# rsmedleystevenson/pyamg

Hardware: AMD Instinct MI355X
Metric: V-cycle iterations/sec (3D Poisson 500^3 fp64, SA-AMG, chebyshev smoother) (higher is better)
Workload: dtype f64; 1 GPU; 3D Poisson 500x500x500 (125.0M dof, nnz 873.5M) CSR fp64, smoothed aggregation (5 levels), Chebyshev degree 2 pre/post smoother, V(1,1), b=rand seed 0; parallelism=single GPU

## Files before the change

include/amgcore_hip.h:

```cpp
#ifndef AMGCORE_HIP_H
#define AMGCORE_HIP_H

#ifdef __cplusplus
extern "C" {
#endif

#define AMG_OK        0
#define AMG_EINVAL   -1
#define AMG_ENODEV   -2
#define AMG_ENOMEM   -3
#define AMG_ESTATE   -4
#define AMG_ENOTIMPL -5

const char *amg_last_error(void);
int amg_device_count(void);
const char *amg_device_name(int device);



int amgcore_gauss_seidel_f64(const int Ap[], int Ap_size, const int Aj[], int Aj_size,
                             const double Ax[], int Ax_size, double x[], int x_size,
                             const double b[], int b_size,
                             int row_start, int row_stop, int row_step);
int amgcore_bsr_gauss_seidel_f64(const int Ap[], int Ap_size, const int Aj[], int Aj_size,
// ... 150 lines not shown
int amg_hier_set_matrix(amg_hier *h, int lvl, int which, int fmt, int nrows, int ncols,
                        int R, int C, const int *Ap, const int *Aj, const double *Ax,
                        int on_device);
int amg_hier_set_smoother(amg_hier *h, int lvl, int which, const amg_smoother_desc *d);
int amg_hier_set_block_matrix(amg_hier *h, int lvl, int which, int nbrows, int bs, const int *Ap,
                              const int *Aj, const double *Ax);
int amg_hier_set_aux_matrix(amg_hier *h, int lvl, int which, int slot, int nmajor, int nminor,
                            const int *Ap, const int *Aj, const double *Ax);
int amg_hier_set_coarse_dense(amg_hier *h, const double *M, int n);
int amg_hier_set_coarse_smoother(amg_hier *h, const amg_smoother_desc *d);
int amg_hier_set_callback_smoother(amg_hier *h, int lvl, int which, amg_relax_callback cb, void *user);
int amg_hier_set_coarse_callback(amg_hier *h, amg_coarse_callback cb, void *user);
int amg_hier_apply(amg_hier *h, int lvl, int which, const double *x_dev, double *y_dev);
int amg_hier_apply_aux(amg_hier *h, int lvl, int which, int slot, const double *x_dev, double *y_dev);
double *amg_hier_scratch(amg_hier *h);
int amg_hier_finalize(amg_hier *h);
long amg_hier_release_sources(amg_hier *h);

int amg_hier_solve(amg_hier *h, const double *b, double *x, double tol, int maxiter, int cycle,
                   double *residuals, int *nres, int flags);
int amg_hier_pcg(amg_hier *h, const double *b, double *x, double tol, int maxiter, int cycle,
                 double *residuals, int *nres, int *info, int flags);
int amg_hier_cycle(amg_hier *h, const double *b, double *x, int cycle, int flags);
int amg_hier_relax(amg_hier *h, int lvl, int which, const double *b, double *x);
int amg_hier_matvec(amg_hier *h, int lvl, int which, const double *x, double *y);

double amg_hier_cycle_bytes(amg_hier *h, int cycle);
int amg_hier_operator_form(amg_hier *h, int lvl);
int amg_hier_value_index(amg_hier *h, int lvl, int on);
void amg_set_value_index(int on);
int amg_value_index_enabled(void);
void amg_set_level0_fusion(int on);
int amg_hier_level0_fused(amg_hier *h);
int amg_hier_gs_natural(amg_hier *h, int lvl, double *x, const double *b, const unsigned char *dirs, int nsweeps);

double amg_hier_operator_bytes(amg_hier *h, int lvl, int moved);
double amg_hier_cycle_bytes_moved(amg_hier *h, int cycle);
double amg_hier_last_solve_ms(amg_hier *h);
long amg_hier_device_bytes(amg_hier *h);
void *amg_hier_stream(amg_hier *h);
double *amg_hier_dev_x(amg_hier *h);
double *amg_hier_dev_b(amg_hier *h);

int amg_hier_time_spmv(amg_hier *h, int lvl, int which, int mode, int reps, double *ms);
int amg_hier_time_relax(amg_hier *h, int lvl, int which, int reps, double *ms);

typedef struct amg_mat amg_mat;
amg_mat *amg_mat_create(int device, int nrows, int ncols, const int *Ap, const int *Aj, const double *Ax);
void amg_mat_destroy(amg_mat *m);
long amg_mat_nnz(amg_mat *m);
int amg_mat_form(amg_mat *m);
int amg_mat_apply(amg_mat *m, int mode, const double *xg, const double *b, const double *v2, double *out,
                  double *out2, double c0, double gscale, void *stream);
int amg_mat_apply_rows(amg_mat *m, int mode, int row_lo, int row_hi, const double *xg, const double *b,
                       const double *v2, double *out, double *out2, double c0, double gscale, void *stream);
int amg_mat_build_gs(amg_mat *m, const int *order, int norder);
int amg_mat_gs_levels(amg_mat *m);
int amg_mat_gs_sweep(amg_mat *m, double *x, const double *b, int reverse, int bsr1, void *stream);
int amg_mat_gs_sweeps(amg_mat *m, double *x, const double *b, const unsigned char *seq, int nseq, int bsr1, void *stream);
int amg_dev_scale(double *out, const double *in, double c, long n, void *stream);
int amg_dev_axpy(double *x, const double *h, long n, void *stream);
int amg_dev_axpy_scaled(double *x, const double *r, double c, long n, void *stream);
int amg_dev_norm2(const double *x, long n, double *scratch, double *result_dev, void *stream);
int amg_dev_dot(const double *x, const double *y, long n, double *scratch, double *result_dev, void *stream);
int amg_dev_dense_apply(const double *Mt, const double *b, double *x, int n, void *stream);
int amg_dev_gather(double *out, const double *in, const int *idx, long n, void *stream);
// ... 146 lines not shown
```

pyamg_amd/_lib.py:

```python
import ctypes as C
import os

import numpy as np

HERE = os.path.dirname(os.path.abspath(__file__))
LIB_PATH = os.environ.get("AMGCORE_HIP_LIB") or os.path.join(HERE, "lib", "libamgcore_hip.so")

c_int_p = C.POINTER(C.c_int)
c_dbl_p = C.POINTER(C.c_double)

AMG_OK, AMG_EINVAL, AMG_ENODEV, AMG_ENOMEM, AMG_ESTATE, AMG_ENOTIMPL = 0, -1, -2, -3, -4, -5


class AmgError(RuntimeError):
    pass


class AmgDeviceError(AmgError):
    pass


RELAX_CALLBACK = C.CFUNCTYPE(C.c_int, C.c_void_p, C.c_int, C.c_void_p, C.c_void_p)
COARSE_CALLBACK = C.CFUNCTYPE(C.c_int, C.c_void_p, C.c_int, c_dbl_p, c_dbl_p)

# ... 179 lines not shown
    L.amg_hier_destroy.restype = None
    L.amg_hierx_destroy.argtypes = [V]
    L.amg_hierx_destroy.restype = None
    L.amg_hierx_device_bytes.argtypes = [V]
    L.amg_hierx_device_bytes.restype = C.c_long
    L.amg_hierx_last_solve_ms.argtypes = [V]
    L.amg_hierx_last_solve_ms.restype = D
    L.amg_hierx_stream.argtypes = [V]
    L.amg_hierx_stream.restype = V
    L.amg_hierx_scratch.argtypes = [V]
    L.amg_hierx_scratch.restype = V
    L.amg_hierx_level_size.argtypes = [V, I]
    L.amg_hierx_level_size.restype = I
    L.amg_hierx_vec_alloc.argtypes = [V, C.c_long]
    L.amg_hierx_vec_alloc.restype = V
    L.amg_hierx_vec_free.argtypes = [V, V, C.c_long]
    L.amg_hierx_vec_free.restype = None
    L.amg_hierm_destroy.argtypes = [V]
    L.amg_hierm_destroy.restype = None
    L.amg_hierm_device_bytes.argtypes = [V]
    L.amg_hierm_device_bytes.restype = C.c_long
    L.amg_hierm_last_solve_ms.argtypes = [V]
    L.amg_hierm_last_solve_ms.restype = D
    L.amg_hier_cycle_bytes.argtypes = [V, I]
    L.amg_hier_cycle_bytes.restype = D
    L.amg_hier_value_index.argtypes = [V, I, I]
    L.amg_hier_value_index.restype = I
    L.amg_set_value_index.argtypes = [I]
    L.amg_set_value_index.restype = None
    L.amg_set_level0_fusion.argtypes = [I]
    L.amg_set_level0_fusion.restype = None
    L.amg_hier_level0_fused.argtypes = [V]
    L.amg_hier_level0_fused.restype = I
    L.amg_value_index_enabled.argtypes = []
    L.amg_value_index_enabled.restype = I
    L.amg_hier_gs_natural.argtypes = [V, I, V, V, V, I]
    L.amg_hier_gs_natural.restype = I
    L.amg_hier_operator_form.argtypes = [V, I]
    L.amg_hier_operator_form.restype = I
    L.amg_hier_operator_bytes.argtypes = [V, I, I]
    L.amg_hier_operator_bytes.restype = D
    L.amg_hier_cycle_bytes_moved.argtypes = [V, I]
    L.amg_hier_cycle_bytes_moved.restype = D
    L.amg_hier_last_solve_ms.argtypes = [V]
    L.amg_hier_last_solve_ms.restype = D
    L.amg_hier_device_bytes.argtypes = [V]
    L.amg_hier_device_bytes.restype = C.c_long
    L.amg_hier_stream.argtypes = [V]
    L.amg_hier_stream.restype = V
    L.amg_hier_dev_x.argtypes = [V]
    L.amg_hier_dev_x.restype = V
    L.amg_hier_dev_b.argtypes = [V]
    L.amg_hier_dev_b.restype = V
    L.amg_dev_alloc.argtypes = [C.c_long]
    L.amg_dev_alloc.restype = V
    L.amg_dev_free.argtypes = [V]
    L.amg_dev_free.restype = None
    L.amg_hier_scratch.argtypes = [V]
    L.amg_hier_scratch.restype = V
    L.amg_comm_create.argtypes = [I, I, I, I]
    L.amg_comm_create.restype = V
    L.amg_comm_destroy.argtypes = [V]
    L.amg_comm_destroy.restype = None
    L.amg_hier_release_sources.argtypes = [V]
    L.amg_hier_release_sources.restype = C.c_long
    L.amg_mat_create.argtypes = [I, I, I, c_int_p, c_int_p, c_dbl_p]
# ... 77 lines not shown
```

pyamg_amd/csrc/amg_dev.hpp:

```cpp
#pragma once
#include <hip/hip_runtime.h>
#include <cstdint>
#include <string>
#include <vector>

namespace amg {

void set_error(const std::string &msg);
int hip_fail(hipError_t e, const char *what, const char *file, int line);
#define AMG_HIP(call)                                                         \
    do {                                                                      \
        hipError_t e__ = (call);                                              \
        if (e__ != hipSuccess) return amg::hip_fail(e__, #call, __FILE__, __LINE__); \
    } while (0)

constexpr int PAD = 16;

struct DevBsr;
struct DevCsr {
    int nrows = 0, ncols = 0;
    long nnz = 0;
    int *Ap = nullptr;
    int *Aj = nullptr;
    double *Ax = nullptr;
// ... 6 lines not shown
    int npat = 0, ndict = 0;
    int period_rows = 0;
    int *sl_row = nullptr;
    unsigned short *sl_len = nullptr;
    long *sl_off = nullptr;
    int *sl_col = nullptr;
    double *sl_val = nullptr;
    int sl_nslices = 0;
    unsigned *sl_code = nullptr;
    int *sl_org = nullptr;
    long *sl_coff = nullptr;
    unsigned char *sl_flag16 = nullptr;
    double sl_frac16 = 0.0;
    long sl_entries = 0;
    int sl_lo = 0, sl_hi = 0;
    double *st_vals = nullptr;
    void *st_mask = nullptr;
    int st_nu = 0;
    int st_nranges = 0;
    int st_range[8][2] = {{0}};
    unsigned char *st_codes = nullptr;
    double *st_dict = nullptr;
    int st_ndict = 0;
    bool st_vi_on = false;
    unsigned short *Aj16 = nullptr;
    int *wg_base = nullptr;
    unsigned char *wg_flag = nullptr;
    int i16_rpb = 0;
    double i16_frac = 0.0;
    int st_u0 = -1;
    int st_off[32] = {0};
    int l0_ok = 0;
    int l0_nx = 0, l0_ny = 0, l0_nz = 0;
};
constexpr int STENCIL_MAX = 31;
constexpr int STENCIL_RANGES = 8;

constexpr int PAT_MAX = 255;
constexpr int PAT_DICT_MAX = 2048;

struct DevBsr {
    int nbrows = 0, bs = 1;
    long nblocks = 0;
    int *Ap = nullptr;
    int *Aj = nullptr;
    double *Ax = nullptr;
    int *bsl_brow = nullptr;
    unsigned short *bsl_len = nullptr;
    long *bsl_off = nullptr;
    int *bsl_col = nullptr;
    double *bsl_val = nullptr;
    int bsl_nslices = 0;
};

enum StreamMode {
    SM_MATVEC = 0,
    SM_MATVEC_ACC,
    SM_RESIDUAL,
    SM_POLY_FIRST,
    SM_POLY_STEP,
    SM_POLY_LAST,
    SM_JACOBI,
    SM_JACOBI_BSR1,
    SM_GS,
    SM_GS_BSR1,
    SM_RESIDUAL_SUMSQ,
// ... 15 lines not shown
    long nnz_total;
    int rows_per_wg;
    const unsigned short *Aj16;
    const int *wg_base;
    const unsigned char *wg_flag;
    double gscale;
};

int launch_stream(StreamMode mode, const StreamArgs &a, hipStream_t st);
int launch_pattern(StreamMode mode, const StreamArgs &a, const DevCsr &M, hipStream_t st);
bool pattern_supports(StreamMode mode);
int launch_stencil(StreamMode mode, const StreamArgs &a, const DevCsr &M, hipStream_t st);
bool sell_supports(StreamMode mode);
bool sell_enabled();
void set_sell_form(int on);
void set_sell_index16(int on);
bool sell_index16_enabled();
int launch_sell(StreamMode mode, const StreamArgs &a, const DevCsr &M, hipStream_t st);
int build_sell(DevCsr &M, long *acct, int row_lo = 0, int row_hi = -1);
void free_sell(DevCsr &M);
int stencil_blocks(const StreamArgs &a, const DevCsr &M);
struct Level0ChainArgs {
    const unsigned long long *codes;
    const double *dict;
    int ndict;
    int nx, ny, nz;
    const double *g0;
    const double *x;
    const double *b;
    double *xout, *rout;
    double c_gs, c_last;
    int zc;
    int tiles_x, tiles_y;
};
int launch_level0_chain(bool first_res, bool last_res, const Level0ChainArgs &a, hipStream_t st);
int level0_chain_tile(int stages, int axis);
int level0_chain_lanes(int axis);
int launch_sumsq_partials(const double *r, int n, double *out2, hipStream_t st);
int launch_level0_box_scan(const unsigned char *codes, int nx, int ny, int nz, int *bad, hipStream_t st);
int launch_stencil_build(const DevCsr &M, const int *dict_slot, const unsigned *pat_mask, hipStream_t st);
int launch_value_scan(const double *vals, long count, unsigned long long *table, int *overflow, hipStream_t st);
int launch_value_encode(const double *vals, long count, const double *dict_sorted, int ndict, unsigned char *codes, int nu,
                        hipStream_t st, const unsigned char *mask8 = nullptr, long nrows = 0);
int config_epoch();
void bump_config_epoch();
int launch_gs_chain(const DevCsr &G, const int *rowmap, const int *diagpos, const int *level_ptr_dev, int l_first,
                    int nlevels, int width, bool reverse, bool bsr1, double *x, const double *b, hipStream_t st);
constexpr int CHAIN2_WG = 512;
constexpr int CHAIN2_PF = 12;
constexpr int CHAIN2_D = 2;
constexpr int CHAIN2_LMAX = 4096;
constexpr int CHAIN2_EMPTY = -2147483647 - 1;
int launch_perm_gather(const int *rowmap, const double *x, const double *b, const double *diag, double *xp, double *bp, double *bd,
                       int n, hipStream_t st);
int launch_perm_scatter(const int *rowmap, const double *xp, double *x, int n, hipStream_t st);
int launch_gs_chain2(const int *lp, const double *val, const int *code, const int *off, double *dummy, int pf,
                     int l_first, int nlevels, int width, bool reverse, bool bsr1, double *x, const double *bd, int nzero, hipStream_t st);
int gs_chain_max_rows();
int launch_gs_chain_long(const DevCsr &G, const int *rowmap, const int *diagpos, const int *level_ptr_dev, int l_first,
                         int nlevels, int width, bool reverse, bool bsr1, double *x, const double *b, hipStream_t st,
                         const int *ring_code = nullptr);
int gs_chainl_max_levels();
int launch_gs_level(const StreamArgs &a, bool bsr1, const int *gp_host, hipStream_t st);
void set_gs_level_hint(int on);
int gs_chainl_max_rows();
int gs_chainl_entries_per_lane();
bool gs_chain_enabled();
int gs_chain_generation();
void set_gs_chain(int on);
bool stencil_enabled();
int launch_index16_build(DevCsr &M, int rpb, hipStream_t st);
bool index16_enabled();
// ... 115 lines not shown
```

pyamg_amd/csrc/hier.hip:

```cpp
#include <array>
#include <thread>
#include "hier.hpp"

#include <algorithm>
#include <cmath>
#include <cstdlib>
#include <cstring>

namespace amg {

static thread_local std::string g_err;
void set_error(const std::string &msg) { g_err = msg; }
const std::string &last_error() { return g_err; }
int hip_fail(hipError_t e, const char *what, const char *file, int line)
{
    g_err = std::string("HIP error: ") + hipGetErrorString(e) + " in " + what + " (" + file + ":" +
            std::to_string(line) + ")";
    return (e == hipErrorOutOfMemory) ? AMG_ENOMEM : AMG_ENODEV;
}

#define CHK(call)                 \
    do {                          \
        int rc__ = (call);        \
        if (rc__ != 0) return rc__; \
    } while (0)

template <class T> static int dev_alloc(T **p, long count, long *acct)
{
    size_t bytes = sizeof(T) * (size_t)(count + PAD);
    AMG_HIP(hipMalloc((void **)p, bytes));
    AMG_HIP(hipMemset(*p, 0, bytes));
    AMG_HIP(hipDeviceSynchronize());
    if (acct) *acct += (long)bytes;
    return 0;
}

void free_csr(DevCsr &M)
{
    if (M.Ap) hipFree(M.Ap);
    if (M.Aj) hipFree(M.Aj);
    if (M.Ax) hipFree(M.Ax);
    if (M.pat) hipFree(M.pat);
    if (M.dict_ptr) hipFree(M.dict_ptr);
    if (M.dict_off) hipFree(M.dict_off);
    free_sell(M);
    if (M.st_vals) hipFree(M.st_vals);
    if (M.st_mask) hipFree(M.st_mask);
    if (M.st_codes) hipFree(M.st_codes);
    if (M.st_dict) hipFree(M.st_dict);
    if (M.Aj16) hipFree(M.Aj16);
    if (M.wg_base) hipFree(M.wg_base);
    if (M.wg_flag) hipFree(M.wg_flag);
    M = DevCsr();
}
static void free_bsr(DevBsr &M)
{
    free_bsell(M);
    if (M.Ap) hipFree(M.Ap);
    if (M.Aj) hipFree(M.Aj);
    if (M.Ax) hipFree(M.Ax);
    M = DevBsr();
}

int upload_csr(DevCsr &M, int nrows, int ncols, const int *Ap, const int *Aj, const double *Ax,
               long *acct)
{
    long nnz = Ap[nrows];
    if (nnz < 0 || nrows < 0) { set_error("row pointer overflows int32 (more than 2^31-1 stored entries)"); return AMG_EINVAL; }
    M.nrows = nrows; M.ncols = ncols; M.nnz = nnz;
    CHK(dev_alloc(&M.Ap, nrows + 1, acct));
    CHK(dev_alloc(&M.Aj, nnz, acct));
    CHK(dev_alloc(&M.Ax, nnz, acct));
    AMG_HIP(hipMemcpy(M.Ap, Ap, sizeof(int) * (size_t)(nrows + 1), hipMemcpyHostToDevice));
    if (nnz) {
        AMG_HIP(hipMemcpy(M.Aj, Aj, sizeof(int) * (size_t)nnz, hipMemcpyHostToDevice));
        AMG_HIP(hipMemcpy(M.Ax, Ax, sizeof(double) * (size_t)nnz, hipMemcpyHostToDevice));
    }
    return 0;
}

int build_index16(DevCsr &M, const int *Ap_host, long *acct)
{
// ... 1087 lines not shown
}

static int coarse_solve(amg_hier *h, const double *b, double *&x, double *&xalt)
{
    Level &L = h->lv[h->nlevels - 1];
    const int n = L.A.nrows;
    if (L.A.nnz == 0 || h->coarse_kind == 0) {
        AMG_HIP(hipMemsetAsync(x, 0, sizeof(double) * (size_t)n, h->stream));
        return 0;
    }
    if (h->coarse_kind == 1 && h->comm && h->coarse_gather_channel >= 0) {
        CHK(comm_exchange_begin(h->comm, h->coarse_gather_channel, b, h->coarse_gather_idx, h->coarse_full_b, h->stream));
        CHK(comm_exchange_end(h->comm, h->coarse_gather_channel, h->coarse_full_b, h->stream));
        CHK(launch_dense_apply(h->coarse_Mt, h->coarse_full_b, h->coarse_full_x, h->coarse_n, h->stream));
        AMG_HIP(hipMemcpyAsync(x, h->coarse_full_x + h->coarse_lo, sizeof(double) * (size_t)n, hipMemcpyDeviceToDevice, h->stream));
        return 0;
    }
    if (h->coarse_kind == 1) return launch_dense_apply(h->coarse_Mt, b, x, n, h->stream);
    if (h->coarse_kind == 3) {
        h->coarse_hb.resize((size_t)n); h->coarse_hx.assign((size_t)n, 0.0);
        AMG_HIP(hipMemcpyAsync(h->coarse_hb.data(), b, sizeof(double) * (size_t)n, hipMemcpyDeviceToHost, h->stream));
        AMG_HIP(hipStreamSynchronize(h->stream));
        if (h->coarse_cb(h->coarse_cb_user, n, h->coarse_hb.data(), h->coarse_hx.data()) != 0) { set_error("coarse solver callback failed"); return AMG_ESTATE; }
        AMG_HIP(hipMemcpyAsync(x, h->coarse_hx.data(), sizeof(double) * (size_t)n, hipMemcpyHostToDevice, h->stream));
        AMG_HIP(hipStreamSynchronize(h->stream));
        return 0;
    }
    if (h->comm && L.part.channel >= 0) { set_error("relaxation as coarse solver has no row-partitioned form"); return AMG_ENOTIMPL; }
    AMG_HIP(hipMemsetAsync(x, 0, sizeof(double) * (size_t)n, h->stream));
    return relax(h, L, h->coarse_sm, x, xalt, b, true);
}

static int g_level0_fusion = 1;
#ifndef L0_ZCHUNK_PLANES
#define L0_ZCHUNK_PLANES 128
#endif
constexpr int L0_ZCHUNK = L0_ZCHUNK_PLANES;

static int level0_chain_check(amg_hier *h, DevCsr &M)
{
    M.l0_ok = 0;
    if (!M.st_vals || !M.st_codes || M.st_nu != 7 || M.st_nranges != 0 || M.nrows != M.ncols || M.nrows < 1) return 0;
    const int *o = M.st_off;
    const long n = M.nrows, Lx = o[5], P = o[6];
    if (!(o[0] == -P && o[1] == -Lx && o[2] == -1 && o[3] == 0 && o[4] == 1)) return 0;
    if (!(Lx > 1 && P > Lx && P % Lx == 0 && n % P == 0)) return 0;
    int *bad = nullptr;
    if (dev_alloc(&bad, 1, nullptr) != 0) return AMG_ENOMEM;
    int found = 1;
    int rc = 0;
    if (hipMemsetAsync(bad, 0, sizeof(int), h->stream) != hipSuccess) rc = AMG_ESTATE;
    if (rc == 0) rc = launch_level0_box_scan(M.st_codes, (int)Lx, (int)(P / Lx), (int)(n / P), bad, h->stream);
    if (rc == 0 && (hipMemcpyAsync(&found, bad, sizeof(int), hipMemcpyDeviceToHost, h->stream) != hipSuccess ||
                    hipStreamSynchronize(h->stream) != hipSuccess)) rc = AMG_ESTATE;
    hipFree(bad);
    if (rc != 0) return rc;
    if (found) return 0;
    M.l0_nx = (int)Lx; M.l0_ny = (int)(P / Lx); M.l0_nz = (int)(n / P);
    M.l0_ok = 1;
    return 0;
}

static bool level0_fused(amg_hier *h)
{
    if (!g_level0_fusion || h->comm || h->nlevels < 2) return false;
    const Level &L = h->lv[0];
    const DevCsr &M = L.A;
    if (!M.l0_ok || !M.st_vi_on || !M.st_codes || (M.blk && M.blk->Ap) || !(stencil_enabled() || !M.Ap)) return false;
    for (int w = 0; w < 2; ++w) {
        const Smoother &s = L.sm[w];
        if (s.kind != AMG_SM_POLYNOMIAL || s.coef.size() != 2 || s.iterations != 1) return false;
    }
    return true;
}

static int level0_chain(amg_hier *h, const Smoother &s, bool first_res, bool last_res, const double *g0, double *&x,
                        double *&xalt, const double *b, double *rout)
{
    const DevCsr &M = h->lv[0].A;
    Level0ChainArgs a{};
    a.codes = reinterpret_cast<const unsigned long long *>(M.st_codes);
    a.dict = M.st_dict; a.ndict = M.st_ndict;
    a.nx = M.l0_nx; a.ny = M.l0_ny; a.nz = M.l0_nz;
    a.g0 = g0; a.x = x; a.b = b; a.xout = xalt; a.rout = rout;
    a.c_gs = s.coef[0]; a.c_last = s.coef[1];
    a.zc = std::min(L0_ZCHUNK, M.l0_nz);
    CHK(launch_level0_chain(first_res, last_res, a, h->stream));
    std::swap(x, xalt);
    return 0;
}

static int level0_pre_chain(amg_hier *h, double *&x, double *&xalt, const double *b, bool x_zero, bool r_ready)
{
    Level &L = h->lv[0];
    if (x_zero) return level0_chain(h, L.sm[AMG_PRE], false, true, b, x, xalt, b, L.h);
    if (r_ready) return level0_chain(h, L.sm[AMG_PRE], false, true, L.r, x, xalt, b, L.h);
    return level0_chain(h, L.sm[AMG_PRE], true, true, x, x, xalt, b, L.h);
}

static int level0_post_chain(amg_hier *h, double *&x, double *&xalt, const double *b)
{
    Level &L = h->lv[0];
    const bool norm = h->norm_next;
    CHK(level0_chain(h, L.sm[AMG_POST], true, norm, x, x, xalt, b, norm ? L.r : nullptr));
    h->r_fresh = norm;
    return 0;
}

static int cycle(amg_hier *h, int lvl, double *&x, double *&xalt, const double *b, int cyc, bool x_zero,
                 bool r_ready = false)
{
    Level &L = h->lv[lvl];
    Level &Lc = h->lv[lvl + 1];
    hipStream_t st = h->stream;
    const int nc = Lc.A.nrows;
    const bool fused = lvl == 0 && level0_fused(h);

    double *rr = L.r;
    if (fused) {
// ... 1131 lines not shown
        const double f16 = (M.sl_code && sell_index16_enabled()) ? M.sl_frac16 : 0.0;
        return (12.0 - 2.0 * f16) * (double)M.sl_entries + (6.0 * 64.0 + 64.0 * f16 + 1.0) * M.sl_nslices + 8.0 * (M.sl_nslices + 1.0) + 8.0 * M.ncols + 8.0 * M.nrows;
    }
    if (!M.pat) {
        double idx = (M.Aj16 && index16_enabled()) ? (2.0 * M.i16_frac + 4.0 * (1.0 - M.i16_frac)) : 4.0;
        return (8.0 + idx) * (double)M.nnz + 4.0 * (M.nrows + 1.0) + 8.0 * M.ncols + 8.0 * M.nrows;
    }
    return 8.0 * (double)M.nnz + 4.0 * M.nrows + 4.0 * (M.nrows + 1.0) + 8.0 * M.ncols + 8.0 * M.nrows;
}

static double cycle_bytes_impl(amg_hier *h, int cyc, bool moved)
{
    if (!h) return 0.0;
    std::vector<double> visits((size_t)h->nlevels, 0.0);
    visits[0] = 1.0;
    for (int l = 1; l < h->nlevels; ++l) {
        if (cyc == AMG_CYCLE_W) visits[l] = 2.0 * visits[l - 1];
        else if (cyc == AMG_CYCLE_F) visits[l] = visits[l - 1] + 1.0;
        else visits[l] = 1.0;
    }
    double total = 0.0;
    for (int l = 0; l < h->nlevels - 1; ++l) {
        Level &L = h->lv[l];
        double n = L.A.nrows;
        double app = (moved ? bytes_spmv_moved(L.A) : bytes_spmv(L.A)) + 8.0 * n;
        double k = smoother_apps(L.sm[0], l > 0) + 1.0 + smoother_apps(L.sm[1], false);
        double extra = 0.0;
        if (l == 0 && moved && level0_fused(h)) {
            const double zc = std::min(L0_ZCHUNK, L.A.l0_nz);
            const double tx = level0_chain_lanes(0), ty = level0_chain_lanes(1);
            auto chain = [&](int S, int row_operands, int outputs) {
                const double in = (double)level0_chain_tile(S, 0) * level0_chain_tile(S, 1);
                const double zf = (zc + 2.0 * S) / zc;
                return 8.0 * n * (tx * ty / in * zf + row_operands * (tx - 2.0) * (ty - 2.0) / in * zf + outputs);
            };
            const bool kept = h->keep_residual != 0;
            const double pre = kept ? chain(2, 3, 2) : chain(3, 2, 2);
            const double post = chain(3, 2, 2) + 8.0 * n;
            total += visits[l] * (pre + post + bytes_spmv(L.Rm) + bytes_spmv(L.P) + 8.0 * n);
            continue;
        }
        if (l == 0) {
            k += 1.0;
            if (moved && h->keep_residual && L.sm[0].kind == AMG_SM_POLYNOMIAL && L.sm[0].iterations >= 1) {
                k -= 1.0;
                extra = 8.0 * n;
            }
        }
        total += visits[l] * (k * app + extra + bytes_spmv(L.Rm) + bytes_spmv(L.P) + 8.0 * n);
    }
    double ncs = h->lv[h->nlevels - 1].A.nrows;
    total += visits[h->nlevels - 1] * (8.0 * ncs * ncs + 16.0 * ncs);
    return total;
}

int amg_hier_value_index(amg_hier *h, int lvl, int on)
{
    ENTER(h);
    if (lvl < 0 || lvl >= h->nlevels) { set_error("bad level"); return AMG_EINVAL; }
    DevCsr &M = h->lv[lvl].A;
    if (on < 0) return (M.st_vi_on && M.st_codes) ? M.st_ndict : 0;
    drop_graphs(h);
    if (!on) { M.st_vi_on = false; return 0; }
    return value_index_build(h, M);
}

int amg_hier_operator_form(amg_hier *h, int lvl)
{
    if (!h || lvl < 0 || lvl >= h->nlevels) return -1;
    const DevCsr &M = h->lv[lvl].A;
    if (M.st_vals && (stencil_enabled() || !M.Ap)) return 2;
// ... 268 lines not shown
    Level &L = h->lv[lvl];
    Smoother &s = (which == 2) ? h->coarse_sm : L.sm[which];
    CHK(relax(h, L, s, L.x, L.xalt, L.b, false));
    AMG_HIP(hipEventRecord(h->ev0, h->stream));
    for (int r = 0; r < reps; ++r) CHK(relax(h, L, s, L.x, L.xalt, L.b, false));
    AMG_HIP(hipEventRecord(h->ev1, h->stream));
    AMG_HIP(hipStreamSynchronize(h->stream));
    float t = 0.f;
    AMG_HIP(hipEventElapsedTime(&t, h->ev0, h->ev1));
    *ms = t / reps;
    return 0;
}

void amg_set_stream_variant(int v) { amg::set_stream_variant(v); }
void amg_set_stream_pipe(int on) { amg::set_stream_pipe(on); }
void amg_set_xcd_chunk(int c) { amg::set_xcd_chunk(c); }
void amg_set_xcd_period(int on) { amg::set_xcd_period(on); }
void amg_set_stencil_form(int on) { amg::set_stencil_form(on); }
void amg_set_stencil_pairs(int on) { amg::set_stencil_pairs(on); }
void amg_set_sell_form(int on) { amg::set_sell_form(on); }
void amg_set_sell_index16(int on) { amg::set_sell_index16(on); }
void amg_set_gs_chain(int on) { amg::set_gs_chain(on); }
void amg_set_gs_level_hint(int on) { amg::set_gs_level_hint(on); }
void amg_set_gs_flow(int mode) { amg::set_gs_flow(mode); }
void amg_set_gs_flow_lookahead(int levels) { amg::set_gs_flow_lookahead(levels); }
int amg_gs_flow_status(void) { return amg::gs_flow_status(); }
void amg_set_bsr_spmv(int on) { amg::set_bsr_spmv(on); }
void amg_set_index16(int on) { amg::set_index16(on); }
void amg_set_tile_target(int t) { amg::set_tile_target(t); }
void amg_hier_use_graphs(amg_hier *h, int on) { if (h) { h->use_graphs = on; if (!on) drop_graphs(h); } }
void amg_hier_keep_residual(amg_hier *h, int on) { if (h) { h->keep_residual = on; h->r_kept = false; drop_graphs(h); } }
void amg_set_level0_fusion(int on) { g_level0_fusion = on ? 1 : 0; amg::bump_config_epoch(); }
int amg_hier_level0_fused(amg_hier *h) { return (h && h->finalized && level0_fused(h)) ? 1 : 0; }

}
```

pyamg_amd/csrc/kernels.hip:

```cpp
#include "amg_dev.hpp"

namespace amg {

constexpr int WG = 256;
#ifndef AMG_TILE
#define AMG_TILE 2048
#endif
constexpr int TILE = AMG_TILE;

typedef int v4i __attribute__((ext_vector_type(4)));
typedef double v2d __attribute__((ext_vector_type(2)));
__device__ __forceinline__ v4i load_v4i(const int *p)
{
#ifdef AMG_NT_LOADS
    return __builtin_nontemporal_load(reinterpret_cast<const v4i *>(p));
#else
    return *reinterpret_cast<const v4i *>(p);
#endif
}
__device__ __forceinline__ v2d load_v2d(const double *p)
{
#ifdef AMG_NT_LOADS
    return __builtin_nontemporal_load(reinterpret_cast<const v2d *>(p));
#else
    return *reinterpret_cast<const v2d *>(p);
#endif
}

static int g_stream_variant = 1;
static int g_xcd_chunk = 32;
static int g_tile_target = 2048;
static int g_config_epoch = 0;
int config_epoch() { return g_config_epoch; }
// ... 1856 lines not shown
        c.row_hi = std::min(a.row_hi, M.st_range[r][1]);
        if (c.row_hi <= c.row_lo) continue;
        if (MODE == SM_RESIDUAL_SUMSQ) c.out2 = a.out2 + done;
        int rc = launch_pattern((StreamMode)MODE, c, M, st);
        if (rc != 0) return rc;
        done += (c.row_hi - c.row_lo + rpb - 1) / rpb;
    }
    return 0;
}

int launch_stencil(StreamMode mode, const StreamArgs &a, const DevCsr &M, hipStream_t st)
{
    switch (mode) {
    case SM_MATVEC: return launch_stencil_mode<SM_MATVEC>(a, M, st);
    case SM_MATVEC_ACC: return launch_stencil_mode<SM_MATVEC_ACC>(a, M, st);
    case SM_RESIDUAL: return launch_stencil_mode<SM_RESIDUAL>(a, M, st);
    case SM_POLY_STEP: return launch_stencil_mode<SM_POLY_STEP>(a, M, st);
    case SM_POLY_LAST: return launch_stencil_mode<SM_POLY_LAST>(a, M, st);
    case SM_JACOBI: return launch_stencil_mode<SM_JACOBI>(a, M, st);
    case SM_JACOBI_BSR1: return launch_stencil_mode<SM_JACOBI_BSR1>(a, M, st);
    case SM_RESIDUAL_SUMSQ: return launch_stencil_mode<SM_RESIDUAL_SUMSQ>(a, M, st);
    default: break;
    }
    set_error("launch_stencil: mode not supported");
    return -1;
}

#ifndef L0C_TY
#define L0C_TY 16
#endif
constexpr int L0C_TX = 32;
constexpr int L0C_WG = L0C_TX * L0C_TY;
constexpr int L0C_PAD = L0C_TX;

template <int FR, int LR>
__global__ __launch_bounds__(L0C_WG) void level0_chain_kernel(Level0ChainArgs a)
{
    constexpr int S = FR + 1 + LR;
    constexpr int SP = FR + 1;
    constexpr int INX = L0C_TX - 2 * S, INY = L0C_TY - 2 * S;
    __shared__ double sdict[256];
    __shared__ double pl[2][S][L0C_WG + 2 * L0C_PAD];
    const int t = threadIdx.x, tx = t % L0C_TX, ty = t / L0C_TX;
    const int bid = remap_block(blockIdx.x, gridDim.x, 16);
    const int tiles = a.tiles_x * a.tiles_y;
    const int zb = bid / tiles, rem = bid - zb * tiles;
    const int tyi = rem / a.tiles_x, txi = rem - tyi * a.tiles_x;
    const int gx = txi * INX - S + tx, gy = tyi * INY - S + ty;
    const bool inxy = gx >= 0 && gx < a.nx && gy >= 0 && gy < a.ny;
    const bool ring1 = inxy && tx >= 1 && tx < L0C_TX - 1 && ty >= 1 && ty < L0C_TY - 1;
    const bool inner = inxy && tx >= S && tx < L0C_TX - S && ty >= S && ty < L0C_TY - S;
    const long P = (long)a.nx * a.ny;
    const long col = inxy ? (long)gy * a.nx + gx : 0;
    const int z0 = zb * a.zc, z1 = min(z0 + a.zc, a.nz);
    if (t < a.ndict) sdict[t] = a.dict[t];

    double w[S + 1][3];
    unsigned long long cq[S];
    double bq[S];
#pragma unroll
    for (int s = 0; s <= S; ++s) w[s][0] = w[s][1] = w[s][2] = 0.0;
#pragma unroll
    for (int s = 0; s < S; ++s) { cq[s] = ~0ULL; bq[s] = 0.0; }
    double xq = 0.0;
    int k = z0 - S;
    double g_next = (inxy && k >= 0) ? a.g0[(long)k * P + col] : 0.0;
    unsigned long long c_next = ~0ULL;
    double b_next = 0.0, x_next = 0.0;
    const int iters = (z1 - z0) + 2 * S;
    for (int j = 0; j < iters; ++j, ++k) {
        w[0][0] = w[0][1]; w[0][1] = w[0][2]; w[0][2] = g_next;
#pragma unroll
        for (int s = S - 1; s > 0; --s) { cq[s] = cq[s - 1]; bq[s] = bq[s - 1]; }
        cq[0] = c_next; bq[0] = b_next; xq = x_next;
        {
            const int kn = k + 1;
            g_next = (inxy && kn >= 0 && kn < a.nz) ? a.g0[(long)kn * P + col] : 0.0;
            const bool rowk = ring1 && k >= 0 && k < a.nz;
            const long ik = (long)k * P + col;
            c_next = rowk ? a.codes[ik] : ~0ULL;
            b_next = rowk ? a.b[ik] : 0.0;
            if (!FR) x_next = rowk ? a.x[ik] : 0.0;
        }
        double (*plb)[L0C_WG + 2 * L0C_PAD] = pl[j & 1];
#pragma unroll
        for (int s = 1; s <= S; ++s) plb[s - 1][L0C_PAD + t] = s == 1 ? w[0][1] : w[s - 1][2];
        __syncthreads();
#pragma unroll
        for (int s = 1; s <= S; ++s) {
            const double *q = &plb[s - 1][L0C_PAD + t];
            const double xv[7] = {w[s - 1][0], q[-L0C_TX], q[-1], w[s - 1][1], q[1], q[L0C_TX], w[s - 1][2]};
            double diag = 0.0, val;
            if (s == SP) {
                const double acc = coded_row_sum<SM_POLY_LAST>(cq[s - 1], sdict, xv, a.c_gs, true, 0.0, -1, diag);
                val = poly_last_row(a.c_last, w[s - 1][1], acc, FR ? w[0][0] : xq);
            } else {
                const double acc = coded_row_sum<SM_RESIDUAL>(cq[s - 1], sdict, xv, 1.0, true, 0.0, -1, diag);
                val = residual_row(bq[s - 1], acc);
            }
            w[s][0] = w[s][1]; w[s][1] = w[s][2]; w[s][2] = val;
        }
        const int p = k - S;
        if (inner && p >= z0 && p < z1) {
            const long i = (long)p * P + col;
            if (LR) store_out(&a.rout[i], w[S][2]);
            store_out(&a.xout[i], w[SP][2 - (S - SP)]);
        }
    }
}

int level0_chain_tile(int stages, int axis) { return (axis == 0 ? L0C_TX : L0C_TY) - 2 * stages; }
int level0_chain_lanes(int axis) { return axis == 0 ? L0C_TX : L0C_TY; }

int launch_level0_chain(bool first_res, bool last_res, const Level0ChainArgs &a0, hipStream_t st)
{
    Level0ChainArgs a = a0;
    const int S = 1 + (first_res ? 1 : 0) + (last_res ? 1 : 0);
    if (S < 2 || a.nx < 1 || a.ny < 1 || a.nz < 1 || a.zc < 1) { set_error("launch_level0_chain: bad chain"); return -1; }
    const int inx = level0_chain_tile(S, 0), iny = level0_chain_tile(S, 1);
    a.tiles_x = (a.nx + inx - 1) / inx;
    a.tiles_y = (a.ny + iny - 1) / iny;
    const long grid = (long)a.tiles_x * a.tiles_y * ((a.nz + a.zc - 1) / a.zc);
    if (grid > 2147483647L) { set_error("launch_level0_chain: grid too large"); return -1; }
    if (first_res && last_res) hipLaunchKernelGGL((level0_chain_kernel<1, 1>), dim3(grid), dim3(L0C_WG), 0, st, a);
    else if (first_res) hipLaunchKernelGGL((level0_chain_kernel<1, 0>), dim3(grid), dim3(L0C_WG), 0, st, a);
    else hipLaunchKernelGGL((level0_chain_kernel<0, 1>), dim3(grid), dim3(L0C_WG), 0, st, a);
    hipError_t e = hipGetLastError();
    if (e != hipSuccess) return hip_fail(e, "level-0 chain launch", __FILE__, __LINE__);
    return 0;
}

constexpr int SSQ_BLOCKS = 2;
__global__ __launch_bounds__(WG) void sumsq_partials_kernel(const double *r, int n, int nb, double *out2)
{
// ... 25 lines not shown
int launch_sumsq_partials(const double *r, int n, double *out2, hipStream_t st)
{
    if (n <= 0) return 0;
    const int nb = (n + WG - 1) / WG;
    const int per_wg = SSQ_BLOCKS * (WG / 64);
    hipLaunchKernelGGL(sumsq_partials_kernel, dim3((nb + per_wg - 1) / per_wg), dim3(WG), 0, st, r, n, nb, out2);
    hipError_t e = hipGetLastError();
    if (e != hipSuccess) return hip_fail(e, "sumsq partials launch", __FILE__, __LINE__);
    return 0;
}

__global__ void level0_box_scan_kernel(const unsigned long long *codes, int nx, int ny, int nz, int *bad)
{
    const long n = (long)nx * ny * nz;
    for (long i = blockIdx.x * (long)blockDim.x + threadIdx.x; i < n; i += (long)gridDim.x * blockDim.x) {
        const unsigned long long cw = codes[i];
        const int x = (int)(i % nx);
        const long r = i / nx;
        const int y = (int)(r % ny), z = (int)(r / ny);
        const bool ok[7] = {z > 0, y > 0, x > 0, true, x < nx - 1, y < ny - 1, z < nz - 1};
        bool fail = false;
#pragma unroll
        for (int u = 0; u < 7; ++u) fail |= ((unsigned)(cw >> (8 * u)) & 0xFFu) != 255u && !ok[u];
        if (fail) *bad = 1;
    }
}

int launch_level0_box_scan(const unsigned char *codes, int nx, int ny, int nz, int *bad, hipStream_t st)
{
    hipLaunchKernelGGL(level0_box_scan_kernel, dim3(4096), dim3(256), 0, st, reinterpret_cast<const unsigned long long *>(codes),
                       nx, ny, nz, bad);
    hipError_t e = hipGetLastError();
    if (e != hipSuccess) return hip_fail(e, "level-0 box scan launch", __FILE__, __LINE__);
    return 0;
}

__global__ __launch_bounds__(WG) void index16_build_kernel(int nrows, int rpb, const int *Ap, const int *Aj,
                                                          unsigned short *Aj16, int *wg_base, unsigned char *wg_flag)
{
    __shared__ int sset[16];
    __shared__ int sover;
    const int t = threadIdx.x, wg = blockIdx.x;
    const int r0 = wg * rpb;
    const int nr = min(rpb, nrows - r0);
    const int kbeg = Ap[r0], kend = Ap[r0 + nr];
    if (t < 16) sset[t] = -1;
    if (t == 0) sover = 0;
    __syncthreads();
    for (int k = kbeg + t; k < kend; k += WG) {
        const int w = Aj[k] >> 12;
        bool placed = false;
        for (int s = 0; s < 16 && !placed; ++s) {
            int cur = atomicCAS(&sset[s], -1, w);
            placed = (cur == -1 || cur == w);
        }
        if (!placed) sover = 1;
    }
    __syncthreads();
    if (sover) {
        if (t == 0) wg_flag[wg] = 0;
        return;
    }
    for (int k = kbeg + t; k < kend; k += WG) {
        const int c = Aj[k], w = c >> 12;
        int slot = 0;
        for (int s = 0; s < 16; ++s) if (sset[s] == w) slot = s;
// ... 780 lines not shown
```

Baseline: 91.35 V-cycle iterations/s.

## Skip stencil code loads and decoding for fully interior level-0 tile planes

At setup, the code precomputes per-tile, per-z-plane bitflags marking planes whose coded rows all equal the canonical interior 7-point stencil word. In the fused level-0 Chebyshev chain kernel, flagged planes skip loading the 8-byte code word per row. When every stage in the pipeline is interior, the kernel uses a constant-coefficient 7-term sum instead of dictionary decoding. This cuts level-0 memory traffic and decode ALU work, at the cost of a setup kernel, small flag arrays, and a branch plus extra registers in the hot kernel.

```diff
diff --git a/include/amgcore_hip.h b/include/amgcore_hip.h
--- a/include/amgcore_hip.h
+++ b/include/amgcore_hip.h
@@ -206,6 +206,8 @@
 int amg_value_index_enabled(void);
 void amg_set_level0_fusion(int on);
 int amg_hier_level0_fused(amg_hier *h);
+void amg_set_level0_interior(int on);
+long amg_hier_level0_interior_planes(amg_hier *h, int stages);
 int amg_hier_gs_natural(amg_hier *h, int lvl, double *x, const double *b, const unsigned char *dirs, int nsweeps);
 
 double amg_hier_operator_bytes(amg_hier *h, int lvl, int moved);
diff --git a/pyamg_amd/_lib.py b/pyamg_amd/_lib.py
--- a/pyamg_amd/_lib.py
+++ b/pyamg_amd/_lib.py
@@ -235,6 +235,10 @@
     L.amg_set_level0_fusion.restype = None
     L.amg_hier_level0_fused.argtypes = [V]
     L.amg_hier_level0_fused.restype = I
+    L.amg_set_level0_interior.argtypes = [I]
+    L.amg_set_level0_interior.restype = None
+    L.amg_hier_level0_interior_planes.argtypes = [V, I]
+    L.amg_hier_level0_interior_planes.restype = C.c_long
     L.amg_value_index_enabled.argtypes = []
     L.amg_value_index_enabled.restype = I
     L.amg_hier_gs_natural.argtypes = [V, I, V, V, V, I]
diff --git a/pyamg_amd/csrc/amg_dev.hpp b/pyamg_amd/csrc/amg_dev.hpp
--- a/pyamg_amd/csrc/amg_dev.hpp
+++ b/pyamg_amd/csrc/amg_dev.hpp
@@ -62,6 +62,13 @@
     int st_off[32] = {0};
     int l0_ok = 0;
     int l0_nx = 0, l0_ny = 0, l0_nz = 0;
+    int l0_wstar_ok = 0;
+    unsigned long long l0_wstar = ~0ULL;
+    double l0_coef[7] = {0.0};
+    unsigned *l0_flags[2] = {nullptr, nullptr};
+    long l0_nflag[2] = {0, 0};
+    long l0_nplanes[2] = {0, 0};
+    long l0_nwords[2] = {0, 0};
 };
 constexpr int STENCIL_MAX = 31;
 constexpr int STENCIL_RANGES = 8;
@@ -143,12 +150,17 @@
     double c_gs, c_last;
     int zc;
     int tiles_x, tiles_y;
+    const unsigned *flags;
+    unsigned long long wstar;
+    double coef[7];
 };
 int launch_level0_chain(bool first_res, bool last_res, const Level0ChainArgs &a, hipStream_t st);
 int level0_chain_tile(int stages, int axis);
 int level0_chain_lanes(int axis);
 int launch_sumsq_partials(const double *r, int n, double *out2, hipStream_t st);
 int launch_level0_box_scan(const unsigned char *codes, int nx, int ny, int nz, int *bad, hipStream_t st);
+int launch_level0_interior_flags(const unsigned char *codes, int nx, int ny, int nz, int stages, unsigned long long wstar,
+                                 unsigned *flags, unsigned long long *count, hipStream_t st);
 int launch_stencil_build(const DevCsr &M, const int *dict_slot, const unsigned *pat_mask, hipStream_t st);
 int launch_value_scan(const double *vals, long count, unsigned long long *table, int *overflow, hipStream_t st);
 int launch_value_encode(const double *vals, long count, const double *dict_sorted, int ndict, unsigned char *codes, int nu,
diff --git a/pyamg_amd/csrc/hier.hip b/pyamg_amd/csrc/hier.hip
--- a/pyamg_amd/csrc/hier.hip
+++ b/pyamg_amd/csrc/hier.hip
@@ -48,6 +48,7 @@
     if (M.st_mask) hipFree(M.st_mask);
     if (M.st_codes) hipFree(M.st_codes);
     if (M.st_dict) hipFree(M.st_dict);
+    for (unsigned *f : M.l0_flags) if (f) hipFree(f);
     if (M.Aj16) hipFree(M.Aj16);
     if (M.wg_base) hipFree(M.wg_base);
     if (M.wg_flag) hipFree(M.wg_flag);
@@ -1201,14 +1202,17 @@
 }
 
 static int g_level0_fusion = 1;
+static int g_level0_interior = std::getenv("AMG_L0_INTERIOR") ? (std::atoi(std::getenv("AMG_L0_INTERIOR")) ? 1 : 0) : 1;
 #ifndef L0_ZCHUNK_PLANES
 #define L0_ZCHUNK_PLANES 128
 #endif
 constexpr int L0_ZCHUNK = L0_ZCHUNK_PLANES;
 
+static int level0_interior_build(amg_hier *h, DevCsr &M);
 static int level0_chain_check(amg_hier *h, DevCsr &M)
 {
     M.l0_ok = 0;
+    M.l0_wstar_ok = 0;
     if (!M.st_vals || !M.st_codes || M.st_nu != 7 || M.st_nranges != 0 || M.nrows != M.ncols || M.nrows < 1) return 0;
     const int *o = M.st_off;
     const long n = M.nrows, Lx = o[5], P = o[6];
@@ -1227,7 +1231,49 @@
     if (found) return 0;
     M.l0_nx = (int)Lx; M.l0_ny = (int)(P / Lx); M.l0_nz = (int)(n / P);
     M.l0_ok = 1;
-    return 0;
+    return level0_interior_build(h, M);
+}
+
+static int level0_interior_build(amg_hier *h, DevCsr &M)
+{
+    const long centre = ((long)(M.l0_nz / 2) * M.l0_ny + M.l0_ny / 2) * M.l0_nx + M.l0_nx / 2;
+    unsigned long long w = ~0ULL;
+    double dict[256];
+    AMG_HIP(hipMemcpy(&w, reinterpret_cast<const unsigned long long *>(M.st_codes) + centre, sizeof(w), hipMemcpyDeviceToHost));
+    AMG_HIP(hipMemcpy(dict, M.st_dict, sizeof(dict), hipMemcpyDeviceToHost));
+    for (int u = 0; u < 7; ++u) {
+        const unsigned c = (unsigned)(w >> (8 * u)) & 0xFFu;
+        if (c == 255u) return 0;
+        M.l0_coef[u] = dict[c];
+    }
+    unsigned long long *count = nullptr;
+    if (dev_alloc(&count, 2, nullptr) != 0) return AMG_ENOMEM;
+    int rc = 0;
+    for (int d = 0; d < 2 && rc == 0; ++d) {
+        const int S = d + 2;
+        const long tx = (M.l0_nx + level0_chain_tile(S, 0) - 1) / level0_chain_tile(S, 0);
+        const long ty = (M.l0_ny + level0_chain_tile(S, 1) - 1) / level0_chain_tile(S, 1);
+        const long planes = tx * ty * M.l0_nz;
+        if (planes > 2147483647L) break;
+        const long words = tx * ty * ((M.l0_nz + 31) / 32);
+        if (dev_alloc(&M.l0_flags[d], words, &h->dev_bytes) != 0) { rc = AMG_ENOMEM; break; }
+        M.l0_nplanes[d] = planes; M.l0_nwords[d] = words;
+        rc = launch_level0_interior_flags(M.st_codes, M.l0_nx, M.l0_ny, M.l0_nz, S, w, M.l0_flags[d], count + d, h->stream);
+    }
+    unsigned long long got[2] = {0, 0};
+    if (rc == 0 && (hipMemcpyAsync(got, count, sizeof(got), hipMemcpyDeviceToHost, h->stream) != hipSuccess ||
+                    hipStreamSynchronize(h->stream) != hipSuccess)) rc = AMG_ESTATE;
+    hipFree(count);
+    if (rc != 0) return rc;
+    for (int d = 0; d < 2; ++d) M.l0_nflag[d] = M.l0_flags[d] ? (long)got[d] : 0;
+    M.l0_wstar = w;
+    M.l0_wstar_ok = 1;
+    return 0;
+}
+
+static const unsigned *level0_interior_flags(const DevCsr &M, int S)
+{
+    return (g_level0_interior && M.l0_ok && M.l0_wstar_ok && (S == 2 || S == 3)) ? M.l0_flags[S - 2] : nullptr;
 }
 
 static bool level0_fused(amg_hier *h)
@@ -1254,6 +1300,9 @@
     a.g0 = g0; a.x = x; a.b = b; a.xout = xalt; a.rout = rout;
     a.c_gs = s.coef[0]; a.c_last = s.coef[1];
     a.zc = std::min(L0_ZCHUNK, M.l0_nz);
+    a.flags = level0_interior_flags(M, 1 + (first_res ? 1 : 0) + (last_res ? 1 : 0));
+    a.wstar = M.l0_wstar;
+    for (int u = 0; u < 7; ++u) a.coef[u] = M.l0_coef[u];
     CHK(launch_level0_chain(first_res, last_res, a, h->stream));
     std::swap(x, xalt);
     return 0;
@@ -2451,11 +2500,15 @@
             auto chain = [&](int S, int row_operands, int outputs) {
                 const double in = (double)level0_chain_tile(S, 0) * level0_chain_tile(S, 1);
                 const double zf = (zc + 2.0 * S) / zc;
-                return 8.0 * n * (tx * ty / in * zf + row_operands * (tx - 2.0) * (ty - 2.0) / in * zf + outputs);
+                const bool fl = level0_interior_flags(L.A, S) != nullptr;
+                const double planes = (double)L.A.l0_nplanes[S - 2];
+                const double decoded = fl ? 1.0 - (double)L.A.l0_nflag[S - 2] / planes : 1.0;
+                return 8.0 * n * (tx * ty / in * zf + (row_operands + decoded) * (tx - 2.0) * (ty - 2.0) / in * zf + outputs) +
+                       (fl ? 4.0 * (double)L.A.l0_nwords[S - 2] : 0.0);
             };
             const bool kept = h->keep_residual != 0;
-            const double pre = kept ? chain(2, 3, 2) : chain(3, 2, 2);
-            const double post = chain(3, 2, 2) + 8.0 * n;
+            const double pre = kept ? chain(2, 2, 2) : chain(3, 1, 2);
+            const double post = chain(3, 1, 2) + 8.0 * n;
             total += visits[l] * (pre + post + bytes_spmv(L.Rm) + bytes_spmv(L.P) + 8.0 * n);
             continue;
         }
@@ -2790,5 +2843,12 @@
 void amg_hier_keep_residual(amg_hier *h, int on) { if (h) { h->keep_residual = on; h->r_kept = false; drop_graphs(h); } }
 void amg_set_level0_fusion(int on) { g_level0_fusion = on ? 1 : 0; amg::bump_config_epoch(); }
 int amg_hier_level0_fused(amg_hier *h) { return (h && h->finalized && level0_fused(h)) ? 1 : 0; }
-
-}
+void amg_set_level0_interior(int on) { g_level0_interior = on ? 1 : 0; amg::bump_config_epoch(); }
+long amg_hier_level0_interior_planes(amg_hier *h, int stages)
+{
+    if (!h || h->nlevels < 1 || (stages != 2 && stages != 3)) return -1;
+    const DevCsr &M = h->lv[0].A;
+    return (M.l0_ok && M.l0_wstar_ok) ? M.l0_nflag[stages - 2] : 0;
+}
+
+}
diff --git a/pyamg_amd/csrc/kernels.hip b/pyamg_amd/csrc/kernels.hip
--- a/pyamg_amd/csrc/kernels.hip
+++ b/pyamg_amd/csrc/kernels.hip
@@ -1,4 +1,5 @@
 #include "amg_dev.hpp"
+#include <type_traits>
 
 namespace amg {
 
@@ -1921,6 +1922,24 @@
 constexpr int L0C_TX = 32;
 constexpr int L0C_WG = L0C_TX * L0C_TY;
 constexpr int L0C_PAD = L0C_TX;
+#ifndef L0I_SKIP_LOAD
+#define L0I_SKIP_LOAD 1
+#endif
+#ifndef L0I_FAST_SUM
+#define L0I_FAST_SUM 1
+#endif
+
+template <bool SCALE>
+__device__ __forceinline__ double interior_row_sum(const double (&cv)[7], const double (&xv)[7], double gscale)
+{
+    double acc = 0.0;
+#pragma unroll
+    for (int u = 0; u < 7; ++u) {
+        const double pr = cv[u] * (SCALE ? gscale * xv[u] : xv[u]);
+        acc = acc + pr;
+    }
+    return acc;
+}
 
 template <int FR, int LR>
 __global__ __launch_bounds__(L0C_WG) void level0_chain_kernel(Level0ChainArgs a)
@@ -1953,6 +1972,13 @@
     for (int s = 0; s < S; ++s) { cq[s] = ~0ULL; bq[s] = 0.0; }
     double xq = 0.0;
     int k = z0 - S;
+    typedef const __attribute__((address_space(4))) unsigned *FlagWords;
+    const FlagWords fl = a.flags ? (FlagWords)(a.flags + (long)rem * ((a.nz + 31) >> 5)) : nullptr;
+    auto flag_at = [&](int z) -> unsigned { return (fl && z >= 0 && z < a.nz) ? (fl[z >> 5] >> (z & 31)) & 1u : 0u; };
+    unsigned fq[S], fk = 0;
+#pragma unroll
+    for (int s = 0; s < S; ++s) fq[s] = 0;
+    unsigned f_n1 = flag_at(k), f_n2 = flag_at(k + 1);
     double g_next = (inxy && k >= 0) ? a.g0[(long)k * P + col] : 0.0;
     unsigned long long c_next = ~0ULL;
     double b_next = 0.0, x_next = 0.0;
@@ -1960,14 +1986,17 @@
     for (int j = 0; j < iters; ++j, ++k) {
         w[0][0] = w[0][1]; w[0][1] = w[0][2]; w[0][2] = g_next;
 #pragma unroll
-        for (int s = S - 1; s > 0; --s) { cq[s] = cq[s - 1]; bq[s] = bq[s - 1]; }
+        for (int s = S - 1; s > 0; --s) { cq[s] = cq[s - 1]; bq[s] = bq[s - 1]; fq[s] = fq[s - 1]; }
         cq[0] = c_next; bq[0] = b_next; xq = x_next;
+        fq[0] = fk; fk = f_n1; f_n1 = f_n2;
         {
+            f_n2 = flag_at(k + 2);
             const int kn = k + 1;
             g_next = (inxy && kn >= 0 && kn < a.nz) ? a.g0[(long)kn * P + col] : 0.0;
             const bool rowk = ring1 && k >= 0 && k < a.nz;
             const long ik = (long)k * P + col;
-            c_next = rowk ? a.codes[ik] : ~0ULL;
+            if (L0I_SKIP_LOAD && fk) c_next = rowk ? a.wstar : ~0ULL;
+            else c_next = rowk ? a.codes[ik] : ~0ULL;
             b_next = rowk ? a.b[ik] : 0.0;
             if (!FR) x_next = rowk ? a.x[ik] : 0.0;
         }
@@ -1975,20 +2004,30 @@
 #pragma unroll
         for (int s = 1; s <= S; ++s) plb[s - 1][L0C_PAD + t] = s == 1 ? w[0][1] : w[s - 1][2];
         __syncthreads();
-#pragma unroll
-        for (int s = 1; s <= S; ++s) {
-            const double *q = &plb[s - 1][L0C_PAD + t];
-            const double xv[7] = {w[s - 1][0], q[-L0C_TX], q[-1], w[s - 1][1], q[1], q[L0C_TX], w[s - 1][2]};
-            double diag = 0.0, val;
-            if (s == SP) {
-                const double acc = coded_row_sum<SM_POLY_LAST>(cq[s - 1], sdict, xv, a.c_gs, true, 0.0, -1, diag);
-                val = poly_last_row(a.c_last, w[s - 1][1], acc, FR ? w[0][0] : xq);
-            } else {
-                const double acc = coded_row_sum<SM_RESIDUAL>(cq[s - 1], sdict, xv, 1.0, true, 0.0, -1, diag);
-                val = residual_row(bq[s - 1], acc);
-            }
-            w[s][0] = w[s][1]; w[s][1] = w[s][2]; w[s][2] = val;
-        }
+        auto run_stages = [&](auto interior) {
+            constexpr bool INTERIOR = decltype(interior)::value;
+#pragma unroll
+            for (int s = 1; s <= S; ++s) {
+                const double *q = &plb[s - 1][L0C_PAD + t];
+                const double xv[7] = {w[s - 1][0], q[-L0C_TX], q[-1], w[s - 1][1], q[1], q[L0C_TX], w[s - 1][2]};
+                double diag = 0.0, val, acc;
+                if (s == SP) {
+                    if (INTERIOR) acc = interior_row_sum<true>(a.coef, xv, a.c_gs);
+                    else acc = coded_row_sum<SM_POLY_LAST>(cq[s - 1], sdict, xv, a.c_gs, true, 0.0, -1, diag);
+                    val = poly_last_row(a.c_last, w[s - 1][1], acc, FR ? w[0][0] : xq);
+                } else {
+                    if (INTERIOR) acc = interior_row_sum<false>(a.coef, xv, 1.0);
+                    else acc = coded_row_sum<SM_RESIDUAL>(cq[s - 1], sdict, xv, 1.0, true, 0.0, -1, diag);
+                    val = residual_row(bq[s - 1], acc);
+                }
+                w[s][0] = w[s][1]; w[s][1] = w[s][2]; w[s][2] = val;
+            }
+        };
+        unsigned all_interior = L0I_FAST_SUM;
+#pragma unroll
+        for (int s = 0; s < S; ++s) all_interior &= fq[s];
+        if (all_interior) run_stages(std::true_type());
+        else run_stages(std::false_type());
         const int p = k - S;
         if (inner && p >= z0 && p < z1) {
             const long i = (long)p * P + col;
@@ -2080,6 +2119,42 @@
                        nx, ny, nz, bad);
     hipError_t e = hipGetLastError();
     if (e != hipSuccess) return hip_fail(e, "level-0 box scan launch", __FILE__, __LINE__);
+    return 0;
+}
+
+__global__ __launch_bounds__(WG) void level0_interior_flags_kernel(const unsigned long long *codes, int nx, int ny, int nz, int S,
+                                                                  int tiles_x, unsigned long long wstar, unsigned *flags,
+                                                                  unsigned long long *count)
+{
+    const int inx = L0C_TX - 2 * S, iny = L0C_TY - 2 * S;
+    const long bid = blockIdx.x;
+    const int tile = (int)(bid / nz), z = (int)(bid - (long)tile * nz);
+    const int tyi = tile / tiles_x, txi = tile - tyi * tiles_x;
+    int ok = 1;
+    for (int l = threadIdx.x; l < (L0C_TX - 2) * (L0C_TY - 2); l += WG) {
+        const int ty = 1 + l / (L0C_TX - 2), tx = 1 + l - (ty - 1) * (L0C_TX - 2);
+        const int gx = txi * inx - S + tx, gy = tyi * iny - S + ty;
+        if (gx < 0 || gx >= nx || gy < 0 || gy >= ny) ok = 0;
+        else if (codes[((long)z * ny + gy) * nx + gx] != wstar) ok = 0;
+    }
+    const int all = __syncthreads_and(ok);
+    if (threadIdx.x == 0 && all) {
+        atomicOr(&flags[(long)tile * ((nz + 31) >> 5) + (z >> 5)], 1u << (z & 31));
+        atomicAdd(count, 1ULL);
+    }
+}
+
+int launch_level0_interior_flags(const unsigned char *codes, int nx, int ny, int nz, int stages, unsigned long long wstar,
+                                 unsigned *flags, unsigned long long *count, hipStream_t st)
+{
+    const int tiles_x = (nx + level0_chain_tile(stages, 0) - 1) / level0_chain_tile(stages, 0);
+    const int tiles_y = (ny + level0_chain_tile(stages, 1) - 1) / level0_chain_tile(stages, 1);
+    const long grid = (long)tiles_x * tiles_y * nz;
+    if (grid > 2147483647L) return -1;
+    hipLaunchKernelGGL(level0_interior_flags_kernel, dim3(grid), dim3(WG), 0, st, reinterpret_cast<const unsigned long long *>(codes),
+                       nx, ny, nz, stages, tiles_x, wstar, flags, count);
+    hipError_t e = hipGetLastError();
+    if (e != hipSuccess) return hip_fail(e, "level-0 interior flags launch", __FILE__, __LINE__);
     return 0;
 }
 
```

New measurement: 92.89 V-cycle iterations/s (median of 6 runs). Within noise of the previous version (+1.7%).
